# oadrian/GPUFluidSimulator

Hardware: AMD Instinct MI355X
Metric: particle-steps/sec (higher is better)
Workload: dtype f32; 1 GPU; dam-break C3: 256x256x256 = 16777216 particles, grid 512^3, box 32.0, dt 5e-7, jittered lattice, FLOWING: timed after 6000 run-up steps on the device (+5 warm-up); particles=16777216, parallelism=1 GPU, whole domain, state=flow, runup_steps=6000

## Files before the change

gpufluidsimulator_amd/csrc/sph_capi.hip:

```cpp
#include "sph_common.hpp"

#include <cmath>
#include <cstdarg>
#include <cstdlib>
#include <cstring>
#include <new>

namespace sph {

static thread_local std::string g_err;
static int g_device = 0;

void set_error(const char* fmt, ...) {
    char buf[512];
    va_list ap;
    va_start(ap, fmt);
    vsnprintf(buf, sizeof(buf), fmt, ap);
    va_end(ap);
    g_err = buf;
}

int hip_fail(hipError_t e, const char* what, const char* file, int line) {
    set_error("HIP error %d (%s) at %s:%d: %s", (int)e, hipGetErrorString(e), file, line, what);
    return SPH_E_DEVICE;
// ... 150 lines not shown
    if (!rc && (hipHostMalloc((void**)&c->os_err_host, sizeof(uint32_t), hipHostMallocMapped) != hipSuccess ||
                hipHostGetDevicePointer((void**)&c->os_err_dev, c->os_err_host, 0) != hipSuccess)) {
        set_error("hipHostMalloc(mapped) failed");
        rc = SPH_E_NOMEM;
    }
    if (!rc) {
        *c->os_err_host = 0;
        if (hipMemset(c->os_status, 0, (size_t)512 * c->sort_blocks_cap * sizeof(unsigned long long)) != hipSuccess ||
            hipMemset(c->os_status32, 0, (size_t)512 * c->sort_blocks_cap * sizeof(uint32_t)) != hipSuccess ||
            hipMemset(c->os_tickets, 0, 4 * os_groups * sizeof(uint32_t)) != hipSuccess ||
            hipMemset(c->os_hist, 0, os_groups * 4 * 512 * sizeof(uint32_t)) != hipSuccess ||
            hipMemset(c->keyS, 0, tot * sizeof(uint32_t)) != hipSuccess ||
            hipMemset(c->keyS2, 0, tot * sizeof(uint32_t)) != hipSuccess) {
            set_error("hipMemset failed");
            rc = SPH_E_DEVICE;
        }
    }
    if (!rc) rc = dev_alloc(&c->d_scratch, (size_t)64);
    if (!rc && hipHostMalloc((void**)&c->h_scratch, 64 * sizeof(uint32_t)) != hipSuccess) {
        set_error("hipHostMalloc failed");
        rc = SPH_E_NOMEM;
    }
    if (const char* env = getenv("SPH_BLOCK_ORDER")) {
        int x = 1, z = 1, sh = 4, zd = 1, xr = 1;
        if (sscanf(env, "%d,%d,%d,%d,%d", &x, &z, &sh, &zd, &xr) >= 1) {
            c->order_xcd = x != 0; c->order_ztile = z != 0; if (sh >= 1 && sh <= 10) c->order_strip_sh = (uint32_t)sh;
            c->order_ztile_dens = zd != 0; c->order_xrot = xr != 0;
        }
    }
    if (const char* env = getenv("SPH_PAIR_SMALL_SLOTS")) {
        unsigned long v = 0;
        if (sscanf(env, "%lu", &v) == 1) c->pair_small_slots = v > 0xFFFFFFFFul ? 0xFFFFFFFFu : (uint32_t)v;
    }
    {
        const char* env = getenv("SPH_SORT_MERGE");
        c->sort_merge = !(env && env[0] == '0');
        const size_t nchunks = (size_t)ceil_div(capacity, 64u) + 1, ntiles = nchunks / 256 + 2;
        if (!rc) rc = dev_alloc(&c->mm_mask, nchunks);
        if (!rc) rc = dev_alloc(&c->mm_M64, nchunks);
        if (!rc) rc = dev_alloc(&c->mm_tile_cnt, ntiles);
        if (!rc) rc = dev_alloc(&c->mm_tile_off, ntiles);
        if (!rc) rc = dev_alloc(&c->mm_k0, (size_t)capacity);
        if (!rc) rc = dev_alloc(&c->mm_k1, (size_t)capacity);
        if (!rc) rc = dev_alloc(&c->mm_v1, (size_t)capacity);
        if (!rc) rc = dev_alloc(&c->mm_count, (size_t)1);
        if (!rc) rc = dev_alloc(&c->mm_total, (size_t)1);
        if (!rc && (hipHostMalloc((void**)&c->mm_count_host, 8 * sizeof(uint32_t), hipHostMallocMapped) != hipSuccess ||
                    hipHostGetDevicePointer((void**)&c->mm_count_host_dev, c->mm_count_host, 0) != hipSuccess)) {
            set_error("hipHostMalloc(mapped) failed");
            rc = SPH_E_NOMEM;
        }
        if (!rc) {
            c->mm_count_host[0] = 0;
            c->mm_count_host[1] = 1; c->mm_count_host[2] = 0;
            for (int k = 3; k < 8; k++) c->mm_count_host[k] = 0;
            if (hipMemset(c->mm_tile_cnt, 0, ntiles * sizeof(uint32_t)) != hipSuccess ||
                hipMemset(c->mm_count, 0, sizeof(uint32_t)) != hipSuccess ||
                hipMemset(c->mm_total, 0, sizeof(unsigned long long)) != hipSuccess) {
                set_error("hipMemset failed");
                rc = SPH_E_DEVICE;
            }
        }
    }
    if (!rc && hipMemset(c->cells_base, 0, ((size_t)c->grid.ncells + 2) * sizeof(uint2)) != hipSuccess) {
        set_error("hipMemset(cells) failed");
        rc = SPH_E_DEVICE;
// ... 665 lines not shown
    if (rc) return rc;
    c->have_force = true;
    return SPH_OK;
}

int sph_collide(sph_ctx* c) {
    SPH_REQUIRE(c, SPH_E_INVALID, "null context");
    SPH_REQUIRE(c->stage >= sph_ctx::ST_CELLS && c->cells_valid, SPH_E_STATE, "sph_collide needs sph_build_cells first");
    SPH_HIP(hipSetDevice(c->device));
    PhaseTimer t(c, SPH_PH_COLLISION);
    int rc = launch_force(c, false, true, false, 0.f);
    if (rc) return rc;
    c->have_coll = true;
    return SPH_OK;
}

int sph_integrate(sph_ctx* c, float dt) {
    SPH_REQUIRE(c, SPH_E_INVALID, "null context");
    SPH_REQUIRE(c->have_dens && c->have_force && c->have_coll, SPH_E_STATE,
                "sph_integrate needs sph_density, sph_force and sph_collide first");
    SPH_HIP(hipSetDevice(c->device));
    PhaseTimer t(c, SPH_PH_INTEGRATE);
    int rc = launch_integrate(c, dt);
    if (rc) return rc;
    c->have_force = c->have_coll = false;
    return SPH_OK;
}

int sph_step(sph_ctx* c, float dt, uint32_t n_steps) {
    SPH_REQUIRE(c, SPH_E_INVALID, "null context");
    SPH_HIP(hipSetDevice(c->device));
    for (uint32_t s = 0; s < n_steps; s++) {
        int rc = do_hash(c);
        if (!rc) rc = do_sort(c);
        if (!rc) rc = do_cells(c);
        if (!rc) rc = do_density(c);
        if (rc) return rc;
        {
            PhaseTimer t(c, SPH_PH_FORCE);
            rc = launch_force(c, true, true, true, dt);
            if (rc) return rc;
        }
        c->have_force = c->have_coll = false;
        if (c->timing) { c->timed_steps++; if (c->events.size() > 3 * 4096) timing_collect(c); }
    }
    return SPH_OK;
}

int sph_force_collide_integrate(sph_ctx* c, float dt) {
    SPH_REQUIRE(c, SPH_E_INVALID, "null context");
    SPH_REQUIRE(c->stage >= sph_ctx::ST_CELLS && c->have_dens, SPH_E_STATE,
                "sph_force_collide_integrate needs sph_density first");
    SPH_HIP(hipSetDevice(c->device));
    PhaseTimer t(c, SPH_PH_FORCE);
    int rc = launch_force(c, true, true, true, dt);
    if (rc) return rc;
    c->have_force = c->have_coll = false;
    return SPH_OK;
}

int sph_step_phased(sph_ctx* c, float dt, uint32_t n_steps) {
    for (uint32_t s = 0; s < n_steps; s++) {
        int rc = sph_hash(c);
        if (!rc) rc = sph_sort(c);
        if (!rc) rc = sph_build_cells(c);
        if (!rc) rc = sph_density(c);
        if (!rc) rc = sph_force(c);
        if (!rc) rc = sph_collide(c);
        if (!rc) rc = sph_integrate(c, dt);
        if (rc) return rc;
// ... 100 lines not shown
```

gpufluidsimulator_amd/csrc/sph_common.hpp:

```cpp
#pragma once

#include <hip/hip_runtime.h>

#include <cstdint>
#include <cstdio>
#include <string>
#include <vector>

#include "../../include/sph_hip.h"

namespace sph {

constexpr int WAVE = 64;
#ifndef SPH_SORT_KPT
#define SPH_SORT_KPT 16
#endif
constexpr uint32_t SORT_TILE_KEYS = 256 * SPH_SORT_KPT;
#ifndef SPH_PAIR_SMALL_SLOTS_DEFAULT
#define SPH_PAIR_SMALL_SLOTS_DEFAULT 524288u
#endif
constexpr uint32_t MM_TILE_CHUNKS = 256;

struct GridDesc {
    float box_min[3];
// ... 75 lines not shown
    uint32_t order_strip_sh = 4;

    uint2* cells = nullptr;
    uint2* cells_base = nullptr;
    uint32_t cells_alloc = 0;
    uint32_t cells_lo = 0, cells_hi = 0;
    bool cells_valid = false;
    bool cells_clear_deferred = false;
    bool owned_cells_in_bounds = false, owned_cells_pending = false;
    bool defer_ghost_clear = false, ghost_clear_pending = false;
    uint32_t ghost_clear[4] = {0, 0, 0, 0};
    bool keys_fresh = false;

    uint32_t* k0 = nullptr; uint32_t* v0 = nullptr;
    uint32_t* k1 = nullptr; uint32_t* v1 = nullptr;
    uint32_t* os_hist = nullptr;
    uint32_t* os_base = nullptr;
    uint32_t* os_tickets = nullptr;
    uint32_t* os_tot = nullptr;
    uint32_t os_groups_cap = 0;
    unsigned long long* os_status = nullptr;
    uint32_t* os_status32 = nullptr;
    uint32_t os_epoch = 0;
    uint32_t* os_err_host = nullptr;
    uint32_t* os_err_dev = nullptr;
    uint32_t sort_blocks_cap = 0;
    uint32_t key_bits = 0;
    const uint32_t* last_perm = nullptr;
    bool keep_perm = false;
    bool sort_merge = true;
    bool sort_merge_always = false;
    bool order_valid = false;
    bool last_sort_skipped = false;
    bool host_paced = false;
    uint32_t sort_seq_issued = 0;
    uint32_t scan_seq_issued = 0;
    uint32_t cells_seq_next = 0;
    bool mm_counted_valid = false;
    uint64_t sort_merges = 0, sort_calls = 0, sort_skips = 0;
    uint64_t sort_form_both_until = 0;
    uint64_t sort_forms[3] = {0, 0, 0};
    uint64_t* mm_mask = nullptr;
    uint32_t* mm_M64 = nullptr;
    uint32_t* mm_tile_cnt = nullptr; uint32_t* mm_tile_off = nullptr;
    uint32_t* mm_k0 = nullptr; uint32_t* mm_k1 = nullptr; uint32_t* mm_v1 = nullptr;
    uint32_t* mm_count = nullptr;
    uint32_t* mm_count_host = nullptr;
    uint32_t* mm_count_host_dev = nullptr;
    unsigned long long* mm_total = nullptr;
    bool mm_marked = false;
    bool mm_scanned = false;
    uint32_t* mm_tileL = nullptr;
    uint32_t* mm_tileA = nullptr;
    uint32_t mm_marked_off = 0, mm_marked_n = 0;
    uint32_t* d_scratch = nullptr;
    uint32_t* h_scratch = nullptr;

    enum Stage { ST_LOADED = 0, ST_HASHED, ST_SORTED, ST_CELLS } stage = ST_LOADED;
    bool have_force = false, have_coll = false, have_dens = false;

    bool timing = false;
    std::vector<hipEvent_t> events;
    double ph_ms[SPH_PH_COUNT] = {0};
    uint32_t timed_steps = 0;
};

// ... 2 lines not shown
void set_error(const char* fmt, ...);
void mm_drop_marks(sph_ctx* c);
void mm_scan_marks(sph_ctx* c);
int hip_fail(hipError_t e, const char* what, const char* file, int line);

#define SPH_HIP(call)                                                        \
    do {                                                                     \
        hipError_t e__ = (call);                                             \
        if (e__ != hipSuccess) return sph::hip_fail(e__, #call, __FILE__, __LINE__); \
    } while (0)

#define SPH_REQUIRE(cond, code, ...)          \
    do {                                      \
        if (!(cond)) {                        \
            sph::set_error(__VA_ARGS__);      \
            return (code);                    \
        }                                     \
    } while (0)

int launch_hash(sph_ctx* c);
int launch_reset_lattice(sph_ctx* c, const uint32_t lattice[3], int jitter, const float jitter_dims[3], uint64_t start,
                         uint32_t count);
int launch_sort(sph_ctx* c);
int launch_merge_arrivals(sph_ctx* c, uint32_t n_in, uint32_t n_front = 0);
int launch_cells_clear(sph_ctx* c);
int launch_cells_clear_range(sph_ctx* c, uint32_t lo, uint32_t hi);
int launch_cells_build_range(sph_ctx* c, uint32_t lo, uint32_t hi);
int launch_cells_clear_2ranges(sph_ctx* c, uint32_t lo0, uint32_t hi0, uint32_t lo1, uint32_t hi1);
int launch_cells_build_2ranges(sph_ctx* c, uint32_t lo0, uint32_t hi0, uint32_t lo1, uint32_t hi1);
int launch_cells_build(sph_ctx* c);
constexpr uint32_t CELLS_SPT = 4;
inline uint32_t cells_build_blocks(uint32_t count) { return (count + 256u * CELLS_SPT - 1u) / (256u * CELLS_SPT); }
int launch_density(sph_ctx* c);
int launch_force(sph_ctx* c, bool force, bool collide, bool integrate, float dt);
int launch_density_range(sph_ctx* c, uint32_t lo, uint32_t hi);
int launch_density_hole(sph_ctx* c, uint32_t lo, uint32_t hi, uint32_t hole_lo, uint32_t hole_hi);
int launch_density_dev_range(sph_ctx* c, const uint32_t* range_dev, uint32_t max_count);
int launch_force_dev_range(sph_ctx* c, const uint32_t* range_dev, uint32_t max_count, float dt);
int launch_force_hole(sph_ctx* c, uint32_t lo, uint32_t hi, uint32_t hole_lo, uint32_t hole_hi, bool force, bool collide,
                      bool integrate, float dt, bool mark);
bool force_begin(sph_ctx* c, bool integrate);
int launch_force_range(sph_ctx* c, uint32_t lo, uint32_t hi, bool force, bool collide, bool integrate, float dt, bool mark);
void force_finish(sph_ctx* c, bool integrate, bool mark, float dt);
int set_slab_range(sph_ctx* c, uint32_t z_lo, uint32_t z_hi);
int step_hash(sph_ctx* c);
int step_sort(sph_ctx* c);
int step_cells(sph_ctx* c);
int launch_integrate(sph_ctx* c, float dt);

inline uint32_t ceil_div(uint32_t a, uint32_t b) { return (a + b - 1) / b; }

struct PhaseTimer {
    sph_ctx* c; int phase; hipEvent_t a = nullptr, b = nullptr;
    PhaseTimer(sph_ctx* c_, int ph) : c(c_), phase(ph) {
        if (!c->timing) return;
        if (hipEventCreate(&a) != hipSuccess || hipEventCreate(&b) != hipSuccess) { a = b = nullptr; return; }
        hipEventRecord(a, c->stream);
    }
    ~PhaseTimer() {
        if (!a || !b) return;
        hipEventRecord(b, c->stream);
        c->events.push_back(a);
        c->events.push_back(b);
        c->events.push_back((hipEvent_t)(intptr_t)phase);
    }
};
// ... 4 lines not shown
```

gpufluidsimulator_amd/csrc/sph_pairs.hip:

```cpp
#include "sph_device.hpp"

namespace sph {

#ifndef SPH_PAIR_THREADS
#define SPH_PAIR_THREADS 256
#endif
constexpr int PAIR_THREADS = SPH_PAIR_THREADS;
constexpr int PAIR_WAVES = PAIR_THREADS / WAVE;
#ifndef SPH_DENS_THREADS
#define SPH_DENS_THREADS SPH_PAIR_THREADS
#endif
constexpr int DENS_THREADS = SPH_DENS_THREADS;
constexpr int SMALL_THREADS_PAIR = 128;
static inline bool small_blocks(const sph_ctx* c) { return c->n < c->pair_small_slots; }
constexpr int PIECE = 128;

typedef float v2f __attribute__((ext_vector_type(2)));
typedef const volatile __attribute__((address_space(3))) v2f* lds_v2f_ptr;
typedef const volatile __attribute__((address_space(3))) float* lds_f32_ptr;

__global__ __launch_bounds__(256) void k_cells_clear(const uint32_t* __restrict__ key, uint32_t lo, uint32_t hi,
                                                     uint2* __restrict__ cells) {
    uint32_t s = lo + blockIdx.x * 256u + threadIdx.x;
    if (s >= hi) return;
// ... 236 lines not shown
#pragma clang loop unroll(disable)
    for (int r = 0; r < 9; r++) {
        uint32_t l0, l1;
        lane_row_one(cells, g, key, active, r / 3 - 1, r % 3 - 1, l0, l1);
        const uint32_t len = l1 > l0 ? l1 - l0 : 0u;
        const uint32_t T = wave_max_u32(len);
        if (T) row(l0, len, T);
    }
}

struct Targets {
    uint32_t lo, hi, gap_lo, gap_len;
    const uint32_t* dev;
    uint32_t direct_hull;
    BlockOrder order;
};

__device__ __forceinline__ uint32_t pair_block() {
    const uint32_t rot = max(gridDim.x >> 6, 1u);
    return blockIdx.x < rot ? gridDim.x - rot + blockIdx.x : blockIdx.x - rot;
}

__device__ __forceinline__ bool wave_targets(const Targets& T, uint32_t wave, uint32_t lane, uint32_t& i, uint32_t& hi,
                                             uint32_t& first) {
    uint32_t lo = T.lo;
    hi = T.hi;
    if (T.dev) { lo = T.dev[0]; hi = T.dev[1]; }
    first = lo + (ordered_block(pair_block(), gridDim.x, T.order) * (blockDim.x >> 6) + wave) * WAVE;
    if (first >= T.gap_lo) first += T.gap_len;
    i = first + lane;
    return first < hi;
}

template <int THREADS>
__global__ __launch_bounds__(THREADS, SPH_DENS_OCC) void k_density(const float4* __restrict__ posi,
                                                                   const uint32_t* __restrict__ keyS,
                                                                   const uint2* __restrict__ cells,
                                                                   float2* __restrict__ dp, float2* __restrict__ cw,
                                                                   Targets tg, GridDesc g, Phys ph) {
    static_assert(UNROLL % 2 == 0, "the z-pair walk reads candidates two at a time");
    constexpr int DENS_ENT = lds_ent(THREADS);
    __shared__ float2 s_xy[DENS_ENT];
    __shared__ __attribute__((aligned(8))) float s_z[DENS_ENT];
    __shared__ __attribute__((aligned(8))) float s_zo_[DENS_ENT + 2];
    float* const s_zo = s_zo_ + 2;
    if (tg.dev && tg.dev[0] + ordered_block(pair_block(), gridDim.x, tg.order) * (uint32_t)THREADS >= tg.dev[1]) return;
    for (uint32_t k = threadIdx.x; k < DENS_ENT; k += THREADS) {
        s_xy[k] = make_float2(0.f, 0.f);
        s_z[k] = 0.f;
        s_zo_[k] = 0.f;
        if (k < 2u) s_zo_[DENS_ENT + k] = 0.f;
    }
    __syncthreads();
    const uint32_t wave = threadIdx.x >> 6, lane = threadIdx.x & 63u;
    const uint32_t slice = wave * PIECE;
    uint32_t i, tgt_hi, wave_first;
    if (!wave_targets(tg, wave, lane, i, tgt_hi, wave_first)) return;
    const bool active = i < tgt_hi;
    const uint32_t ii = active ? i : tgt_hi - 1;
    const float4 pi = posi[ii];
    Rows R;
    const uint32_t my_key = keyS[ii];
    lane_rows(cells, g, my_key, active, R);
    Hulls H;
    wave_hulls(R, H);
    float4 q0, q1;
    float acc = 0.f;
    const float h2_v = in_vgpr(ph.h2);
    auto pair_math = [&](float x, float y, float z, bool valid) {
        const float dx = pi.x - x, dy = pi.y - y, dz = pi.z - z;
        float d = fmaxf(fmaf(-dz, dz, fmaf(-dy, dy, fmaf(-dx, dx, h2_v))), 0.f);
        d = valid ? d : 0.f;
        acc = fmaf(d * d, d, acc);
    };
    auto finish = [&]() {
        if (active) {
            float rho = acc * ph.poly6_mass;
            float p = fmaxf(0.f, ph.gas_constant * (rho - ph.rest_density));
            dp[i] = make_float2(rho, p);
            cw[i] = neighbour_terms(ph, rho, p);
        }
    };
    if (wave_has_long_hull(H, my_key, tg.direct_hull)) {
        const uint32_t me = active ? i : tgt_hi - 1u;
        direct_rows(cells, g, keyS[me], active, [&](uint32_t l0, uint32_t len, uint32_t T) {
            for (uint32_t t = 0; t < T; t += 2u) {
                float4 q[2];
#pragma unroll
                for (uint32_t u = 0; u < 2u; u++) q[u] = posi[t + u < len ? l0 + t + u : me];
#pragma unroll
                for (uint32_t u = 0; u < 2u; u++) pair_math(q[u].x, q[u].y, q[u].z, t + u < len);
            }
        });
        finish();
        return;
    }
// ... 660 lines not shown
}

bool force_begin(sph_ctx* c, bool integrate) {
    if (integrate) mm_drop_marks(c);
    return integrate && c->sort_merge && c->order_valid;
}

void force_finish(sph_ctx* c, bool integrate, bool mark, float dt) {
    if (!integrate) return;
    advance_colliders(c, dt);
    float4* t;
    t = c->posi; c->posi = c->posi2; c->posi2 = t;
    t = c->velr; c->velr = c->velr2; c->velr2 = t;
    c->keys_fresh = true;
    if (mark) {
        c->mm_marked = true; c->mm_scanned = false; c->mm_marked_off = c->own_off; c->mm_marked_n = c->n;
        mm_scan_marks(c);
    }
}

int launch_force(sph_ctx* c, bool force, bool collide, bool integrate, float dt) {
    if (c->n == 0) {
        if (integrate) advance_colliders(c, dt);
        return SPH_OK;
    }
    const bool mark = force_begin(c, integrate);
    int rc = launch_force_range(c, c->own_off, c->own_off + c->n, force, collide, integrate, dt, mark);
    if (rc) return rc;
    force_finish(c, integrate, mark, dt);
    return SPH_OK;
}

static int launch_density_targets(sph_ctx* c, const Targets& tg, uint32_t threads) {
    if (threads == 0) return SPH_OK;
    if (c->precision == SPH_PRECISION_MIXED_F16)
        hipLaunchKernelGGL(k_density_h, dim3(ceil_div(threads, PAIR_THREADS)), dim3(PAIR_THREADS), 0, c->stream, c->posi,
                           c->keyS, c->cells, c->dp, c->cw, tg, c->grid, c->phys);
    else if (small_blocks(c))
        hipLaunchKernelGGL(k_density<SMALL_THREADS_PAIR>, dim3(ceil_div(threads, (uint32_t)SMALL_THREADS_PAIR)), dim3(SMALL_THREADS_PAIR), 0, c->stream,
                           c->posi, c->keyS, c->cells, c->dp, c->cw, tg, c->grid, c->phys);
    else
        hipLaunchKernelGGL(k_density<DENS_THREADS>, dim3(ceil_div(threads, (uint32_t)DENS_THREADS)), dim3(DENS_THREADS), 0, c->stream, c->posi,
                           c->keyS, c->cells, c->dp, c->cw, tg, c->grid, c->phys);
    SPH_HIP(hipGetLastError());
    return SPH_OK;
}

int launch_density_hole(sph_ctx* c, uint32_t lo, uint32_t hi, uint32_t hole_lo, uint32_t hole_hi) {
    if (hi <= lo) return SPH_OK;
    uint32_t threads;
    Targets tg = targets_with_hole(lo, hi, hole_lo, hole_hi, threads);
    tg.direct_hull = c->direct_hull;
    const uint32_t bt = c->precision == SPH_PRECISION_MIXED_F16 ? (uint32_t)PAIR_THREADS : (small_blocks(c) ? (uint32_t)SMALL_THREADS_PAIR : (uint32_t)DENS_THREADS);
    tg.order = block_order(c, ceil_div(threads, bt), c->order_ztile_dens);
    return launch_density_targets(c, tg, threads);
}

int launch_density_range(sph_ctx* c, uint32_t lo, uint32_t hi) { return launch_density_hole(c, lo, hi, hi, hi); }

int launch_density_dev_range(sph_ctx* c, const uint32_t* range_dev, uint32_t max_count) {
    const Targets tg{0u, 0u, 0xFFFFFFFFu, 0u, range_dev, c->direct_hull, BlockOrder{0u, 0u, 0u, 0u, 0u}};
    return launch_density_targets(c, tg, max_count);
}

template <class... Sph>
__global__ __launch_bounds__(256) void k_integrate(float4* __restrict__ posi, float4* __restrict__ velr,
                                                   const float2* __restrict__ dp, const float4* __restrict__ fpress,
                                                   const float4* __restrict__ fvisc, const float4* __restrict__ dvel,
// ... 31 lines not shown
```

gpufluidsimulator_amd/csrc/sph_sort.hip:

```cpp
#include "sph_device.hpp"

#include <atomic>
#include <chrono>

namespace sph {

constexpr int SORT_THREADS = 256;
#ifndef SPH_SORT_KPT
#define SPH_SORT_KPT 16
#endif
constexpr int SORT_KPT = SPH_SORT_KPT;
constexpr int SORT_TILE = SORT_THREADS * SORT_KPT;

__global__ __launch_bounds__(256) void k_hash(const float4* __restrict__ posi, uint32_t n, GridDesc g,
                                              uint32_t* __restrict__ keys) {
    uint32_t i = blockIdx.x * 256u + threadIdx.x;
    if (i >= n) return;
    float4 p = posi[i];
    keys[i] = cell_key(g, p.x, p.y, p.z);
}

constexpr int OS_TILE = SORT_TILE;
#ifndef SPH_OS_GROUP
#define SPH_OS_GROUP 16
// ... 588 lines not shown
        __syncthreads();
#pragma unroll
        for (int t = 0; t < SMALL_KPT; t++) {
            const uint32_t i = wbase + t * WAVE + lane;
            const bool mine = (uint32_t)t < R && i < m;
            key[t] = mine ? s_key[i] : 0xFFFFFFFFu;
            val[t] = mine ? s_val[i] : 0u;
        }
    }
#pragma unroll
    for (int t = 0; t < SMALL_KPT; t++) {
        const uint32_t i = wbase + t * WAVE + lane;
        if ((uint32_t)t < R && i < m) { kout[i] = key[t]; vout[i] = val[t]; }
    }
    if (A) {
        const uint32_t ntiles = (n_slots + OS_TILE - 1) / OS_TILE;
        for (uint32_t t = threadIdx.x; t <= ntiles; t += SMALL_THREADS) {
            const uint32_t slot = t * OS_TILE;
            const uint32_t a = t == ntiles ? 0xFFFFFFFFu : A[slot];
            tileA[t] = a;
            tileL[t] = t == ntiles ? m : small_lower_bound(s_key, s_val, m, a, slot, front);
        }
    }
}

__global__ __launch_bounds__(256) void k_reorder(const uint32_t* __restrict__ ks, const uint32_t* __restrict__ vs,
                                                 uint32_t n, const float4* __restrict__ posi,
                                                 const float4* __restrict__ velr, float4* __restrict__ posi_out,
                                                 float4* __restrict__ velr_out, uint32_t* __restrict__ key_out) {
    uint32_t i = blockIdx.x * 256u + threadIdx.x;
    if (i >= n) return;
    uint32_t src = vs[i];
    posi_out[i] = posi[src];
    velr_out[i] = velr[src];
    key_out[i] = ks[i];
}

__device__ __forceinline__ uint32_t ic_hash(uint32_t x) {
    x ^= x >> 16; x *= 0x7FEB352Du; x ^= x >> 15; x *= 0x846CA68Bu; x ^= x >> 16;
    return x;
}

struct LatticeDesc {
    uint32_t nx, ny;
    float box[3], jdim[3];
    float spacing, radius, jit;
    uint32_t seed;
    int jitter;
};

__global__ __launch_bounds__(256) void k_reset_lattice(float4* __restrict__ posi, float4* __restrict__ velr,
                                                       float2* __restrict__ dp, float4* __restrict__ pos_by_index,
                                                       uint64_t start, uint32_t count, LatticeDesc L) {
#pragma clang fp contract(off)
    uint32_t k = blockIdx.x * 256u + threadIdx.x;
    if (k >= count) return;
    const uint64_t idx = start + k;
    const float ia[3] = {(float)(idx % L.nx), (float)((idx / L.nx) % L.ny), (float)(idx / ((uint64_t)L.nx * L.ny))};
    float p[3];
#pragma unroll
    for (int a = 0; a < 3; a++) {
        const float bmin = -L.box[a] / 2.0f;
        float base = (L.spacing * ia[a] + L.radius) + bmin;
        if (L.jitter) {
            uint32_t h = ic_hash((uint32_t)idx * 3u + (uint32_t)a + L.seed * 0x9E3779B9u);
            h = ic_hash(h ^ 0x85EBCA6Bu);
            const float u = (float)(h >> 8) * (1.0f / 16777216.0f);
// ... 254 lines not shown
    const uint32_t a = t == ntiles ? 0xFFFFFFFFu : A[slot];
    tileA[t] = a;
    tileL[t] = t == ntiles ? m : mm_lower_bound(mk, mi, 0u, m, a, slot, front);
}

__device__ __forceinline__ void mm_scatter_body(uint32_t bid, const uint32_t* __restrict__ A, uint32_t n,
                                                const uint64_t* __restrict__ mask, const uint32_t* __restrict__ M64,
                                                const uint32_t* __restrict__ mk, const uint32_t* __restrict__ mi,
                                                const uint32_t* __restrict__ tileL, const float4* __restrict__ posi,
                                                const float4* __restrict__ velr, float4* __restrict__ posi_out,
                                                float4* __restrict__ velr_out, uint32_t* __restrict__ key_out,
                                                uint32_t* __restrict__ perm_out, Front front) {
    const uint32_t i = bid * 256u + threadIdx.x;
    const uint32_t first = __builtin_amdgcn_readfirstlane(i);
    if (first >= n) return;
    const uint32_t lane = threadIdx.x & 63u;
    const uint32_t chunk = first >> 6;
    const uint32_t last = min(first + 63u, n - 1u);
    const uint32_t tile = first / MM_RANK_TILE;
    const uint32_t b0 = tileL[tile], b1 = tileL[tile + 1];
    uint32_t L0 = b0, L1 = b0;
    if (b0 != b1) {
        L0 = mm_lower_bound(mk, mi, b0, b1, A[first], first, front);
        L1 = mm_lower_bound(mk, mi, L0, b1, A[last], last, front);
    }
    if (i >= n) return;
    const uint64_t bits = mask[chunk];
    if ((bits >> lane) & 1ull) return;
    const uint32_t key = A[i];
    const uint32_t before = M64[chunk] + (uint32_t)__popcll(bits & ((1ull << lane) - 1ull));
    const uint32_t L = L0 == L1 ? L0 : mm_lower_bound(mk, mi, L0, L1, key, i, front);
    const uint32_t dst = i - before + L;
    posi_out[dst] = posi[i];
    velr_out[dst] = velr[i];
    key_out[dst] = key;
    if (perm_out) perm_out[dst] = i;
}

__device__ __forceinline__ void mm_place_body(uint32_t bid, uint32_t nblocks, const uint32_t* __restrict__ A, uint32_t n,
                                              uint32_t nchunks, const uint64_t* __restrict__ mask,
                                              const uint32_t* __restrict__ M64, const uint32_t* __restrict__ mk,
                                              const uint32_t* __restrict__ mi, const uint32_t* __restrict__ m_dev,
                                              const uint32_t* __restrict__ tileA, const uint2* __restrict__ cells,
                                              uint32_t slot_base, const float4* __restrict__ posi,
                                              const float4* __restrict__ velr, float4* __restrict__ posi_out,
                                              float4* __restrict__ velr_out, uint32_t* __restrict__ key_out,
                                              uint32_t* __restrict__ perm_out, Front front) {
    const uint32_t m = *m_dev;
    const uint32_t ntiles = (n + MM_RANK_TILE - 1) / MM_RANK_TILE;
    for (uint32_t r = bid * 256u + threadIdx.x; r < m; r += nblocks * 256u) {
        const uint32_t key = mk[r], slot = mi[r];
        uint32_t s, e;
        uint2 ce = make_uint2(0u, 0u);
        if (cells) ce = cells[key];
        if (ce.y > ce.x) {
            s = ce.x - slot_base; e = ce.y - slot_base;
        } else {
            uint32_t lo = 0, hi = ntiles;
            while (lo < hi) { const uint32_t mid = lo + ((hi - lo) >> 1); if (tileA[mid] < key) lo = mid + 1; else hi = mid; }
            uint32_t a = lo ? (lo - 1u) * MM_RANK_TILE : 0u, b = min(lo * MM_RANK_TILE, n);
            while (a < b) { const uint32_t mid = a + ((b - a) >> 1); if (A[mid] < key) a = mid + 1; else b = mid; }
            s = a;
            uint32_t step = 1u, p = s;
            while (p < n && A[p] == key) { p = min(p + step, n); step <<= 1; }
            uint32_t q = p > s ? max(s, p - (step >> 1)) : s;
            a = q; b = p;
            while (a < b) { const uint32_t mid = a + ((b - a) >> 1); if (A[mid] <= key) a = mid + 1; else b = mid; }
            e = a;
        }
        const uint32_t j = slot - front.lo < front.cnt ? s : min(max(slot, s), e);
        uint32_t before = m;
        if ((j >> 6) < nchunks) before = M64[j >> 6] + (uint32_t)__popcll(mask[j >> 6] & ((1ull << (j & 63u)) - 1ull));
        const uint32_t dst = r + (j - before);
        posi_out[dst] = posi[slot];
        velr_out[dst] = velr[slot];
        key_out[dst] = key;
        if (perm_out) perm_out[dst] = slot;
    }
}

__global__ __launch_bounds__(256) void k_mm_move(uint32_t place_blocks, uint32_t* __restrict__ zero_cnt, uint32_t zero_n,
                                                 const uint32_t* __restrict__ A, uint32_t n,
                                                 uint32_t nchunks, const uint64_t* __restrict__ mask,
                                                 const uint32_t* __restrict__ M64, const uint32_t* __restrict__ mk,
                                                 const uint32_t* __restrict__ mi, const uint32_t* __restrict__ m_dev,
                                                 const uint32_t* __restrict__ tileL, const uint32_t* __restrict__ tileA,
                                                 const uint2* __restrict__ cells, uint32_t slot_base,
                                                 const float4* __restrict__ posi, const float4* __restrict__ velr,
                                                 float4* __restrict__ posi_out, float4* __restrict__ velr_out,
                                                 uint32_t* __restrict__ key_out, uint32_t* __restrict__ perm_out, Front front) {
    if (zero_cnt && blockIdx.x * 256u + threadIdx.x < zero_n) zero_cnt[blockIdx.x * 256u + threadIdx.x] = 0u;
    if (blockIdx.x < place_blocks)
        mm_place_body(blockIdx.x, place_blocks, A, n, nchunks, mask, M64, mk, mi, m_dev, tileA, cells, slot_base, posi, velr,
                      posi_out, velr_out, key_out, perm_out, front);
    else
        mm_scatter_body(blockIdx.x - place_blocks, A, n, mask, M64, mk, mi, tileL, posi, velr, posi_out, velr_out, key_out,
                        perm_out, front);
}

static uint32_t merge_grid_for(uint32_t movers_hint, uint32_t n) {
    const uint32_t want = max(ceil_div(2u * movers_hint + 1u, SORT_TILE) + 15u, OS_ONE_GROUP_TILES);
    return min(want, max(ceil_div(n, SORT_TILE), 1u));
}

static void mm_tilescan(sph_ctx* c, uint32_t n, bool counted) {
    const uint32_t nt = ceil_div(ceil_div(n, 64u), MM_TILE_CHUNKS);
    uint32_t seq = 0u;
    if (counted) { if (++c->scan_seq_issued == 0u) c->scan_seq_issued = 1u; seq = c->scan_seq_issued; }
// ... 20 lines not shown

static bool launch_merge_count(sph_ctx* c, uint32_t n) {
    if (c->mm_marked && !(c->mm_marked_off == c->own_off && c->mm_marked_n == n)) mm_drop_marks(c);
    if (!c->mm_marked) {
        hipLaunchKernelGGL(k_mm_mark, dim3(ceil_div(n, 256)), dim3(256), 0, c->stream, c->keyS + c->own_off, c->k0, n,
                           c->mm_mask, c->mm_tile_cnt);
        c->mm_scanned = false;
    }
    bool in_compact = false;
    if (!c->mm_scanned) {
        if (mm_tiles(n) <= MM_FUSED_SCAN_TILES) { in_compact = true; c->mm_counted_valid = false; }
        else mm_tilescan(c, n, true);
    }
    c->mm_marked = false;
    c->mm_scanned = false;
    return in_compact;
}

__global__ __launch_bounds__(256) void k_mm_mark_tail(uint32_t n_old, uint32_t n_tot, uint64_t* __restrict__ mask,
                                                      uint32_t* __restrict__ tile_cnt) {
    const uint32_t chunk = blockIdx.x * 256u + threadIdx.x;
    if (chunk * 64u >= n_tot) return;
    const uint32_t lo = chunk * 64u, hi = min(lo + 64u, n_tot);
    uint64_t m = 0ull;
    if (hi > n_old) {
        const uint32_t first = max(lo, n_old) - lo, cnt = hi - lo;
        m = (cnt == 64u ? ~0ull : ((1ull << cnt) - 1ull)) & ~((1ull << first) - 1ull);
        atomicAdd(&tile_cnt[chunk / MM_TILE_CHUNKS], (uint32_t)__popcll(m));
    }
    mask[chunk] = m;
}

static int launch_sort_merge(sph_ctx* c, uint32_t n, uint32_t n_tot, bool table_live, uint32_t hint, Front front = Front{0u, 0u},
                             bool count_in_compact = false, const uint32_t* ghost_clear = nullptr) {
    const uint32_t* A = c->keyS + c->own_off;
    const uint32_t* B = c->k0;
    const uint32_t nchunks = ceil_div(n_tot, 64u), nt = ceil_div(nchunks, MM_TILE_CHUNKS);
    uint32_t* mk = c->mm_k0; uint32_t* mi = c->v0; uint32_t* mk2 = c->mm_k1; uint32_t* mi2 = c->mm_v1;
    const uint32_t gc[4] = {ghost_clear ? ghost_clear[0] : 0u, ghost_clear ? ghost_clear[1] : 0u, ghost_clear ? ghost_clear[2] : 0u,
                            ghost_clear ? ghost_clear[3] : 0u};
    const uint32_t gc_blocks = ceil_div((gc[1] - gc[0]) + (gc[3] - gc[2]), 256u);
    hipLaunchKernelGGL(k_mm_compact, dim3(nt + gc_blocks), dim3(256), 0, c->stream, c->mm_mask, nchunks, n, c->mm_tile_off,
                       count_in_compact ? c->mm_tile_cnt : (const uint32_t*)nullptr, nt, c->mm_count, c->mm_count_host_dev, c->mm_total, A, B,
                       c->mm_M64, mk, mi, table_live ? c->cells : (uint2*)nullptr, c->keyS, gc[0], gc[1], gc[2], gc[3]);
    SPH_HIP(hipGetLastError());
    SmallTail tail;
    int form = SORT_FORM_BOTH;
    tail.A = A; tail.n_slots = n; tail.front = front; tail.hint = hint; tail.form = &form;
    int rc = radix_sort_pairs(c, n_tot, c->mm_count, merge_grid_for(hint, n_tot), false, mk, mi, mk2, mi2, tail);
    if (rc) return rc;
    if (form != SORT_FORM_SMALL) {
        const uint32_t rank_tiles = ceil_div(n, MM_RANK_TILE) + 1u;
        hipLaunchKernelGGL(k_mm_tile_rank, dim3(ceil_div(rank_tiles, 256u)), dim3(256), 0, c->stream, A, n, mk, mi, c->mm_count,
                           c->mm_tileL, c->mm_tileA, form == SORT_FORM_BOTH, OS_SMALL_MAX, front);
        SPH_HIP(hipGetLastError());
    }
    uint32_t* perm = c->keep_perm ? c->v1 : (uint32_t*)nullptr;
    const float4* ps = c->posi + c->own_off; const float4* vs = c->velr + c->own_off;
    float4* po = c->posi2 + c->gcap; float4* vo = c->velr2 + c->gcap; uint32_t* ko = c->keyS2 + c->gcap;
    const uint32_t place_blocks = min(max(ceil_div(2u * hint + 1u, 256u) + 15u, 512u), 65535u);
    hipLaunchKernelGGL(k_mm_move, dim3(place_blocks + ceil_div(n, 256)), dim3(256), 0, c->stream, place_blocks,
                       count_in_compact ? c->mm_tile_cnt : (uint32_t*)nullptr, nt, A, n, nchunks,
                       c->mm_mask, c->mm_M64, mk, mi, c->mm_count, c->mm_tileL, c->mm_tileA,
                       table_live ? c->cells : (const uint2*)nullptr, c->own_off, ps, vs, po, vo, ko, perm, front);
    SPH_HIP(hipGetLastError());
    c->last_perm = perm;
    return SPH_OK;
}

static int sort_throttle(sph_ctx* c) {
    volatile const uint32_t* hw = c->mm_count_host;
    if ((int32_t)(c->sort_seq_issued - hw[3]) < 4) return SPH_OK;
    const auto t0 = std::chrono::steady_clock::now();
    for (uint32_t spins = 1; (int32_t)(c->sort_seq_issued - hw[3]) >= 4; spins++) {
        __builtin_ia32_pause();
        if ((spins & 0xFFFu) == 0u) {
            const hipError_t q = hipStreamQuery(c->stream);
            if (q == hipSuccess) break;
            if (q != hipErrorNotReady) SPH_HIP(q);
            SPH_REQUIRE(std::chrono::duration<double>(std::chrono::steady_clock::now() - t0).count() < 300.0, SPH_E_DEVICE,
                        "sort: the device has not reached the table build of sort %u after 300 s", c->sort_seq_issued - 3u);
        }
    }
    return SPH_OK;
}

int launch_sort(sph_ctx* c) {
    const uint32_t n = c->n;
    if (n == 0) return SPH_OK;
    const uint32_t nblocks = ceil_div(n, SORT_TILE);
    SPH_REQUIRE(nblocks <= c->sort_blocks_cap, SPH_E_CAPACITY, "sort: %u blocks > capacity %u", nblocks,
                c->sort_blocks_cap);
    if (c->sort_merge && !c->host_paced) { const int rc = sort_throttle(c); if (rc) return rc; }
    c->sort_calls++;
    c->last_sort_skipped = false;
    const bool can_merge = c->sort_merge && c->order_valid;
    const bool table_live = c->cells_clear_deferred && c->cells_valid;
    c->cells_clear_deferred = false;
    const bool ghosts_left = c->ghost_clear_pending && table_live;
    c->ghost_clear_pending = false;
    if (can_merge && (*c->mm_count_host <= n / 8u || c->sort_merge_always)) {
        const bool was_still = *c->mm_count_host == 0u;
        const bool count_in_compact = launch_merge_count(c, n);
        if (was_still && table_live && c->own_off == c->gcap && !count_in_compact) {
            volatile const uint32_t* hw = c->mm_count_host;
            if (c->mm_counted_valid && hw[4] == c->scan_seq_issued && (std::atomic_thread_fence(std::memory_order_acquire), hw[0] == 0u)) {
                c->sort_merges++;
                c->sort_skips++;
                c->last_sort_skipped = true;
                c->last_perm = nullptr;
                c->order_valid = true;
                if (ghosts_left) {
                    const int rc2 = launch_cells_clear_2ranges(c, c->ghost_clear[0], c->ghost_clear[1], c->ghost_clear[2], c->ghost_clear[3]);
                    if (rc2) return rc2;
                    c->cells_lo = c->own_off; c->cells_hi = c->own_off + n;
                }
                return SPH_OK;
            }
        }
        int rc = launch_sort_merge(c, n, n, table_live, *c->mm_count_host, Front{0u, 0u}, count_in_compact,
                                   ghosts_left ? c->ghost_clear : (const uint32_t*)nullptr);
        if (rc) return rc;
        c->sort_merges++;
        if (c->cells_valid && !table_live) {
            rc = launch_cells_clear(c);
            if (rc) return rc;
        }
    } else {
        if (c->cells_valid) {
            int rc = launch_cells_clear(c);
            if (rc) return rc;
        }
        if (c->mm_marked) {
            if (!c->mm_scanned) mm_tilescan(c, c->mm_marked_n, true);
            c->mm_marked = false;
            c->mm_scanned = false;
        } else if (can_merge && (c->sort_calls & 7u) == 0) {
            hipLaunchKernelGGL(k_mm_mark, dim3(ceil_div(n, 256)), dim3(256), 0, c->stream, c->keyS + c->own_off, c->k0, n,
                               c->mm_mask, c->mm_tile_cnt);
            mm_tilescan(c, n, true);
            SPH_HIP(hipGetLastError());
        }
        uint32_t* kin = c->k0; uint32_t* vin = c->v0;
        uint32_t* kout = c->k1; uint32_t* vout = c->v1;
        int rc = radix_sort_pairs(c, n, nullptr, nblocks, true, kin, vin, kout, vout);
        if (rc) return rc;
        hipLaunchKernelGGL(k_reorder, dim3(ceil_div(n, 256)), dim3(256), 0, c->stream, kin, vin, n, c->posi + c->own_off,
                           c->velr + c->own_off, c->posi2 + c->gcap, c->velr2 + c->gcap, c->keyS2 + c->gcap);
        SPH_HIP(hipGetLastError());
        c->last_perm = vin;
    }
    float4* t4;
    t4 = c->posi; c->posi = c->posi2; c->posi2 = t4;
    t4 = c->velr; c->velr = c->velr2; c->velr2 = t4;
    uint32_t* tk = c->keyS; c->keyS = c->keyS2; c->keyS2 = tk;
    c->own_off = c->gcap;
    c->cells_valid = false;
    if (++c->sort_seq_issued == 0u) c->sort_seq_issued = 1u;
    c->cells_seq_next = c->sort_seq_issued;
    if (c->owned_cells_in_bounds) {
        c->owned_cells_pending = true;
        c->cells_seq_next = 0u;
    } else {
        int rc = launch_cells_build_range(c, c->gcap, c->gcap + n);
        if (rc) return rc;
    }
    c->order_valid = true;
    c->cells_lo = c->gcap; c->cells_hi = c->gcap + n; c->cells_valid = true;
    return SPH_OK;
}

int launch_merge_arrivals(sph_ctx* c, uint32_t n_in, uint32_t n_front) {
    const uint32_t n = c->n, n_tot = n + n_in;
    SPH_REQUIRE(c->order_valid && c->cells_valid && c->cells_lo == c->own_off && c->cells_hi == c->own_off + n, SPH_E_STATE,
                "launch_merge_arrivals needs the sorted owned range and its cell table");
    SPH_REQUIRE(ceil_div(n_tot, SORT_TILE) <= c->sort_blocks_cap, SPH_E_CAPACITY, "sort: capacity exceeded");
    mm_drop_marks(c);
    const uint32_t nchunks = ceil_div(n_tot, 64u);
    hipLaunchKernelGGL(k_mm_mark_tail, dim3(ceil_div(nchunks, 256u)), dim3(256), 0, c->stream, n, n_tot, c->mm_mask,
                       c->mm_tile_cnt);
    const uint32_t nt = ceil_div(nchunks, MM_TILE_CHUNKS);
    hipLaunchKernelGGL(k_mm_tilescan, dim3(1), dim3(1024), 0, c->stream, c->mm_tile_cnt, nt, c->mm_tile_off, c->mm_count,
                       c->mm_count_host_dev, (unsigned long long*)nullptr, 0u);
    c->mm_counted_valid = false;
    SPH_HIP(hipGetLastError());
    int rc = launch_sort_merge(c, n, n_tot, true, n_in, Front{n, n_front < n_in ? n_front : n_in});
    if (rc) return rc;
    float4* t4;
    t4 = c->posi; c->posi = c->posi2; c->posi2 = t4;
    t4 = c->velr; c->velr = c->velr2; c->velr2 = t4;
    uint32_t* tk = c->keyS; c->keyS = c->keyS2; c->keyS2 = tk;
    c->own_off = c->gcap;
    c->n = n_tot;
    c->cells_valid = false;
    rc = launch_cells_build_range(c, c->gcap, c->gcap + n_tot);
    if (rc) return rc;
    c->cells_lo = c->gcap; c->cells_hi = c->gcap + n_tot; c->cells_valid = true;
    c->order_valid = true;
    c->keys_fresh = false;
    c->n_glo = c->n_ghi = 0;
    c->stage = sph_ctx::ST_SORTED;
// ... 27 lines not shown
```

Before: 4.328 billion particle-steps/s.

## Defer velocity reorder from sort into density kernel gather

The sort/merge move kernels no longer write the permuted velocity array. Instead they keep the permutation, and the whole-domain density kernel gathers the old velocities through it, overlapping that load with its cell-row setup. This removes a separate velocity write-then-read pass over 16M float4 values. In exchange it adds a scattered read inside density and a flush path for non-whole or error cases, and it forces the permutation buffer to be written on merges.

```diff
diff --git a/gpufluidsimulator_amd/csrc/sph_capi.hip b/gpufluidsimulator_amd/csrc/sph_capi.hip
--- a/gpufluidsimulator_amd/csrc/sph_capi.hip
+++ b/gpufluidsimulator_amd/csrc/sph_capi.hip
@@ -206,6 +206,10 @@
         unsigned long v = 0;
         if (sscanf(env, "%lu", &v) == 1) c->pair_small_slots = v > 0xFFFFFFFFul ? 0xFFFFFFFFu : (uint32_t)v;
     }
+    if (const char* env = getenv("SPH_LAZY_MOVE")) {
+        int v = 1;
+        if (sscanf(env, "%d", &v) == 1) c->lazy_move = v != 0 ? 1 : 0;
+    }
     {
         const char* env = getenv("SPH_SORT_MERGE");
         c->sort_merge = !(env && env[0] == '0');
@@ -937,10 +941,12 @@
     SPH_HIP(hipSetDevice(c->device));
     for (uint32_t s = 0; s < n_steps; s++) {
         int rc = do_hash(c);
+        c->lazy_vel_wanted = c->lazy_move != 0 && !c->slab && c->precision == SPH_PRECISION_F32;
         if (!rc) rc = do_sort(c);
+        c->lazy_vel_wanted = false;
         if (!rc) rc = do_cells(c);
         if (!rc) rc = do_density(c);
-        if (rc) return rc;
+        if (rc) { flush_lazy_vel(c); return rc; }
         {
             PhaseTimer t(c, SPH_PH_FORCE);
             rc = launch_force(c, true, true, true, dt);
diff --git a/gpufluidsimulator_amd/csrc/sph_common.hpp b/gpufluidsimulator_amd/csrc/sph_common.hpp
--- a/gpufluidsimulator_amd/csrc/sph_common.hpp
+++ b/gpufluidsimulator_amd/csrc/sph_common.hpp
@@ -131,6 +131,10 @@
     bool sort_merge_always = false;
     bool order_valid = false;
     bool last_sort_skipped = false;
+    int lazy_move = 1;
+    bool lazy_vel_wanted = false, lazy_vel_pending = false;
+    const uint32_t* lazy_vel_map = nullptr;
+    uint32_t lazy_vel_off = 0;
     bool host_paced = false;
     uint32_t sort_seq_issued = 0;
     uint32_t scan_seq_issued = 0;
@@ -199,6 +203,7 @@
 constexpr uint32_t CELLS_SPT = 4;
 inline uint32_t cells_build_blocks(uint32_t count) { return (count + 256u * CELLS_SPT - 1u) / (256u * CELLS_SPT); }
 int launch_density(sph_ctx* c);
+int flush_lazy_vel(sph_ctx* c);
 int launch_force(sph_ctx* c, bool force, bool collide, bool integrate, float dt);
 int launch_density_range(sph_ctx* c, uint32_t lo, uint32_t hi);
 int launch_density_hole(sph_ctx* c, uint32_t lo, uint32_t hi, uint32_t hole_lo, uint32_t hole_hi);
diff --git a/gpufluidsimulator_amd/csrc/sph_pairs.hip b/gpufluidsimulator_amd/csrc/sph_pairs.hip
--- a/gpufluidsimulator_amd/csrc/sph_pairs.hip
+++ b/gpufluidsimulator_amd/csrc/sph_pairs.hip
@@ -292,12 +292,19 @@
     return first < hi;
 }
 
-template <int THREADS>
+struct VelMove {
+    const float4* __restrict__ vel_old;
+    const uint32_t* __restrict__ map;
+    float4* __restrict__ vel_out;
+    uint32_t base;
+};
+
+template <int THREADS, class... Mv>
 __global__ __launch_bounds__(THREADS, SPH_DENS_OCC) void k_density(const float4* __restrict__ posi,
                                                                    const uint32_t* __restrict__ keyS,
                                                                    const uint2* __restrict__ cells,
                                                                    float2* __restrict__ dp, float2* __restrict__ cw,
-                                                                   Targets tg, GridDesc g, Phys ph) {
+                                                                   Targets tg, GridDesc g, Phys ph, Mv... mv) {
     static_assert(UNROLL % 2 == 0, "the z-pair walk reads candidates two at a time");
     constexpr int DENS_ENT = lds_ent(THREADS);
     __shared__ float2 s_xy[DENS_ENT];
@@ -321,7 +328,14 @@
     const float4 pi = posi[ii];
     Rows R;
     const uint32_t my_key = keyS[ii];
-    lane_rows(cells, g, my_key, active, R);
+    if constexpr (sizeof...(Mv) > 0) {
+        const VelMove& m = (mv, ...);
+        const float4 v = m.vel_old[m.map[ii - m.base]];
+        lane_rows(cells, g, my_key, active, R);
+        if (active) m.vel_out[i] = v;
+    } else {
+        lane_rows(cells, g, my_key, active, R);
+    }
     Hulls H;
     wave_hulls(R, H);
     float4 q0, q1;
@@ -1048,8 +1062,22 @@
 }
 
 static int launch_density_targets(sph_ctx* c, const Targets& tg, uint32_t threads) {
-    if (threads == 0) return SPH_OK;
-    if (c->precision == SPH_PRECISION_MIXED_F16)
+    if (threads == 0) return flush_lazy_vel(c);
+    if (c->lazy_vel_pending) {
+        const bool whole = !tg.dev && tg.gap_len == 0u && tg.lo == c->own_off && tg.hi == c->own_off + c->n &&
+                           c->precision == SPH_PRECISION_F32;
+        if (!whole) { const int rc = flush_lazy_vel(c); if (rc) return rc; }
+    }
+    if (c->lazy_vel_pending) {
+        const VelMove mv{c->velr2 + c->lazy_vel_off, c->lazy_vel_map, c->velr, c->own_off};
+        c->lazy_vel_pending = false;
+        if (small_blocks(c))
+            hipLaunchKernelGGL((k_density<SMALL_THREADS_PAIR, VelMove>), dim3(ceil_div(threads, (uint32_t)SMALL_THREADS_PAIR)),
+                               dim3(SMALL_THREADS_PAIR), 0, c->stream, c->posi, c->keyS, c->cells, c->dp, c->cw, tg, c->grid, c->phys, mv);
+        else
+            hipLaunchKernelGGL((k_density<DENS_THREADS, VelMove>), dim3(ceil_div(threads, (uint32_t)DENS_THREADS)), dim3(DENS_THREADS), 0,
+                               c->stream, c->posi, c->keyS, c->cells, c->dp, c->cw, tg, c->grid, c->phys, mv);
+    } else if (c->precision == SPH_PRECISION_MIXED_F16)
         hipLaunchKernelGGL(k_density_h, dim3(ceil_div(threads, PAIR_THREADS)), dim3(PAIR_THREADS), 0, c->stream, c->posi,
                            c->keyS, c->cells, c->dp, c->cw, tg, c->grid, c->phys);
     else if (small_blocks(c))
diff --git a/gpufluidsimulator_amd/csrc/sph_sort.hip b/gpufluidsimulator_amd/csrc/sph_sort.hip
--- a/gpufluidsimulator_amd/csrc/sph_sort.hip
+++ b/gpufluidsimulator_amd/csrc/sph_sort.hip
@@ -644,7 +644,7 @@
     if (i >= n) return;
     uint32_t src = vs[i];
     posi_out[i] = posi[src];
-    velr_out[i] = velr[src];
+    if (velr_out) velr_out[i] = velr[src];
     key_out[i] = ks[i];
 }
 
@@ -965,7 +965,7 @@
     const uint32_t L = L0 == L1 ? L0 : mm_lower_bound(mk, mi, L0, L1, key, i, front);
     const uint32_t dst = i - before + L;
     posi_out[dst] = posi[i];
-    velr_out[dst] = velr[i];
+    if (velr_out) velr_out[dst] = velr[i];
     key_out[dst] = key;
     if (perm_out) perm_out[dst] = i;
 }
@@ -1006,7 +1006,7 @@
         if ((j >> 6) < nchunks) before = M64[j >> 6] + (uint32_t)__popcll(mask[j >> 6] & ((1ull << (j & 63u)) - 1ull));
         const uint32_t dst = r + (j - before);
         posi_out[dst] = posi[slot];
-        velr_out[dst] = velr[slot];
+        if (velr_out) velr_out[dst] = velr[slot];
         key_out[dst] = key;
         if (perm_out) perm_out[dst] = slot;
     }
@@ -1093,7 +1093,7 @@
 }
 
 static int launch_sort_merge(sph_ctx* c, uint32_t n, uint32_t n_tot, bool table_live, uint32_t hint, Front front = Front{0u, 0u},
-                             bool count_in_compact = false, const uint32_t* ghost_clear = nullptr) {
+                             bool count_in_compact = false, const uint32_t* ghost_clear = nullptr, bool lazy_vel = false) {
     const uint32_t* A = c->keyS + c->own_off;
     const uint32_t* B = c->k0;
     const uint32_t nchunks = ceil_div(n_tot, 64u), nt = ceil_div(nchunks, MM_TILE_CHUNKS);
@@ -1116,9 +1116,9 @@
                            c->mm_tileL, c->mm_tileA, form == SORT_FORM_BOTH, OS_SMALL_MAX, front);
         SPH_HIP(hipGetLastError());
     }
-    uint32_t* perm = c->keep_perm ? c->v1 : (uint32_t*)nullptr;
+    uint32_t* perm = (c->keep_perm || lazy_vel) ? c->v1 : (uint32_t*)nullptr;
     const float4* ps = c->posi + c->own_off; const float4* vs = c->velr + c->own_off;
-    float4* po = c->posi2 + c->gcap; float4* vo = c->velr2 + c->gcap; uint32_t* ko = c->keyS2 + c->gcap;
+    float4* po = c->posi2 + c->gcap; float4* vo = lazy_vel ? (float4*)nullptr : c->velr2 + c->gcap; uint32_t* ko = c->keyS2 + c->gcap;
     const uint32_t place_blocks = min(max(ceil_div(2u * hint + 1u, 256u) + 15u, 512u), 65535u);
     hipLaunchKernelGGL(k_mm_move, dim3(place_blocks + ceil_div(n, 256)), dim3(256), 0, c->stream, place_blocks,
                        count_in_compact ? c->mm_tile_cnt : (uint32_t*)nullptr, nt, A, n, nchunks,
@@ -1160,6 +1160,8 @@
     c->cells_clear_deferred = false;
     const bool ghosts_left = c->ghost_clear_pending && table_live;
     c->ghost_clear_pending = false;
+    const bool lazy_vel = c->lazy_vel_wanted && !c->slab;
+    const uint32_t old_off = c->own_off;
     if (can_merge && (*c->mm_count_host <= n / 8u || c->sort_merge_always)) {
         const bool was_still = *c->mm_count_host == 0u;
         const bool count_in_compact = launch_merge_count(c, n);
@@ -1180,7 +1182,7 @@
             }
         }
         int rc = launch_sort_merge(c, n, n, table_live, *c->mm_count_host, Front{0u, 0u}, count_in_compact,
-                                   ghosts_left ? c->ghost_clear : (const uint32_t*)nullptr);
+                                   ghosts_left ? c->ghost_clear : (const uint32_t*)nullptr, lazy_vel);
         if (rc) return rc;
         c->sort_merges++;
         if (c->cells_valid && !table_live) {
@@ -1207,10 +1209,12 @@
         int rc = radix_sort_pairs(c, n, nullptr, nblocks, true, kin, vin, kout, vout);
         if (rc) return rc;
         hipLaunchKernelGGL(k_reorder, dim3(ceil_div(n, 256)), dim3(256), 0, c->stream, kin, vin, n, c->posi + c->own_off,
-                           c->velr + c->own_off, c->posi2 + c->gcap, c->velr2 + c->gcap, c->keyS2 + c->gcap);
+                           c->velr + c->own_off, c->posi2 + c->gcap, lazy_vel ? (float4*)nullptr : c->velr2 + c->gcap,
+                           c->keyS2 + c->gcap);
         SPH_HIP(hipGetLastError());
         c->last_perm = vin;
     }
+    if (lazy_vel) { c->lazy_vel_pending = true; c->lazy_vel_map = c->last_perm; c->lazy_vel_off = old_off; }
     float4* t4;
     t4 = c->posi; c->posi = c->posi2; c->posi2 = t4;
     t4 = c->velr; c->velr = c->velr2; c->velr2 = t4;
@@ -1228,6 +1232,22 @@
     }
     c->order_valid = true;
     c->cells_lo = c->gcap; c->cells_hi = c->gcap + n; c->cells_valid = true;
+    return SPH_OK;
+}
+
+__global__ __launch_bounds__(256) void k_gather_vel(const uint32_t* __restrict__ map, uint32_t n, const float4* __restrict__ vel_old,
+                                                    float4* __restrict__ vel_out) {
+    const uint32_t i = blockIdx.x * 256u + threadIdx.x;
+    if (i < n) vel_out[i] = vel_old[map[i]];
+}
+
+int flush_lazy_vel(sph_ctx* c) {
+    if (!c->lazy_vel_pending) return SPH_OK;
+    c->lazy_vel_pending = false;
+    if (c->n == 0) return SPH_OK;
+    hipLaunchKernelGGL(k_gather_vel, dim3(ceil_div(c->n, 256)), dim3(256), 0, c->stream, c->lazy_vel_map, c->n,
+                       c->velr2 + c->lazy_vel_off, c->velr + c->own_off);
+    SPH_HIP(hipGetLastError());
     return SPH_OK;
 }
 
```

Measured after the change: 4.377 billion particle-steps/s (median of 6 runs). 1.01x the previous value.
